# georgehuan1994/OpenGL-Ray-Tracing-Framework

Measured on AMD Instinct MI355X. Metric: Mrays/sec + ms/frame, loong_100000 @1920x1080, 1/2/4/8 MI355X, higher is better.
Workload: dtype f32; 1 GPU; C3: loong_100000 copper metallic (north star); 1920x1080, maxBounce 8, BSDF+MIS+env; width=1920, height=1080, tile=32, parallelism=pixel-tiles x1 + frame-end gather, tile_assignment=interleaved t % N, steps_in_flight=1, triangles=100002, bvh_nodes=35346

## Files before the change

opengl-ray-tracing-framework_amd/csrc/hip/rt_dev_report.h:

```cpp

inline bool dev_passes() {
  static const bool on = knob("RT_DEBUG_PASSES") != nullptr;
  return on;
}
inline size_t dev_wave_words(const rt_ctx* c) { return (size_t)c->n_cus * std::max(c->trace_bpc, c->trace_bpc0) * 4 * 8; }
int dev_wave_log(rt_ctx* c, unsigned long long*& log) {
  static unsigned long long* d_wave_log = nullptr;
  if (dev_passes() && !d_wave_log) HIPCHK(c, hipMalloc(&d_wave_log, dev_wave_words(c) * sizeof(unsigned long long)));
  log = dev_passes() ? d_wave_log : nullptr;
  return RT_OK;
}

int dev_finish_report(rt_ctx* c, bool bsdf, dim3 grid, hipStream_t st, const rtd::WFParams& WP, int g, int pass) {
  std::vector<unsigned long long> wave_log(dev_wave_words(c));
  unsigned long long* const d_wave_log = WP.K.wave_log;
  HIPCHK(c, hipMemsetAsync(d_wave_log, 0, wave_log.size() * 8, st));
  hipEvent_t ft0 = take_event(c), ft1 = take_event(c);
  HIPCHK(c, hipEventRecord(ft0, st));
  launch_finish(c, bsdf, grid, st, WP);
  HIPCHK(c, hipGetLastError());
  HIPCHK(c, hipEventRecord(ft1, st));
  HIPCHK(c, hipStreamSynchronize(st));
  float ms = 0.0f;
  HIPCHK(c, hipEventElapsedTime(&ms, ft0, ft1));
  c->event_pool.push_back(ft0);
  c->event_pool.push_back(ft1);
  HIPCHK(c, hipMemcpy(wave_log.data(), d_wave_log, wave_log.size() * 8, hipMemcpyDeviceToHost));
  struct FW { double t0, t1, sh_us; unsigned long long it, sh, paths; double at[3]; unsigned long long it_at[3]; };
  std::vector<FW> fw;
  double tmin = 1e300;
  for (size_t w = 0; w < wave_log.size() / 8; w++) {
    const unsigned long long* e = &wave_log[8 * w];
    if (!e[1]) continue;
    FW f{e[0] / 100.0, e[1] / 100.0, e[3] / 100.0, e[2] & 0xfffffull, (e[2] >> 20) & 0xfffffull, e[2] >> 40, {}, {}};
    for (int q = 0; q < 3; q++) {
      f.at[q] = e[4 + q] ? (double)(e[4 + q] & 0xffffffffull) / 100.0 : -1.0;
      f.it_at[q] = e[4 + q] >> 32;
    }
    fw.push_back(f);
    tmin = std::min(tmin, e[0] / 100.0);
  }
  std::sort(fw.begin(), fw.end(), [](const FW& a, const FW& b) { return a.t1 > b.t1; });
  unsigned long long paths = 0;
  double life = 0.0, tail16 = 0.0, tail4 = 0.0;
  for (const FW& f : fw) {
    paths += f.paths;
    life += f.t1 - f.t0;
    if (f.at[0] >= 0) tail16 += f.t1 - f.t0 - f.at[0];
    if (f.at[1] >= 0) tail4 += f.t1 - f.t0 - f.at[1];
  }
  fprintf(stderr, "[rt] finisher wave time with <= 16 / <= 4 lanes holding a path (list drained): %.3f / %.3f of %.0f "
          "wave-us\n", tail16 / std::max(1.0, life), tail4 / std::max(1.0, life), life);
  fprintf(stderr, "[rt] group %d finisher from pass %d: %.3f ms, %zu waves, %llu paths; wave ends (us after the first "
          "start) 50%% %.1f 90%% %.1f 99%% %.1f 100%% %.1f\n", g, pass, ms, fw.size(), paths,
          fw.empty() ? 0.0 : fw[fw.size() / 2].t1 - tmin, fw.empty() ? 0.0 : fw[fw.size() / 10].t1 - tmin,
          fw.empty() ? 0.0 : fw[fw.size() / 100].t1 - tmin, fw.empty() ? 0.0 : fw[0].t1 - tmin);
  for (size_t k = 0; k < std::min<size_t>(6, fw.size()); k++) {
    const FW& f = fw[k];
    fprintf(stderr, "[rt]   wave: start %.1f end %.1f us, %llu paths, %llu trace iterations (%.2f us each outside "
            "shade), %llu shade steps %.1f us (%.2f us each); <=16 / 4 / 1 busy lanes from %.0f / %.0f / %.0f us "
            "(iteration %llu / %llu / %llu)\n", f.t0 - tmin, f.t1 - tmin, f.paths, f.it,
            (f.t1 - f.t0 - f.sh_us) / (double)std::max(1ull, f.it), f.sh, f.sh_us, f.sh_us / (double)std::max(1ull, f.sh),
            f.at[0], f.at[1], f.at[2], f.it_at[0], f.it_at[1], f.it_at[2]);
  }
  return RT_OK;
}

int dev_pass_report(rt_ctx* c, hipStream_t st, const rtd::WFParams& WP, int g, int pass, hipEvent_t t0, hipEvent_t t1) {
  unsigned long long h[16];
  unsigned int q[8];
  HIPCHK(c, hipStreamSynchronize(st));
  float ms = 0.0f;
  HIPCHK(c, hipEventElapsedTime(&ms, t0, t1));
  HIPCHK(c, hipMemcpy(h, c->d_stats, sizeof(h), hipMemcpyDeviceToHost));
  HIPCHK(c, hipMemcpy(q, WP.S.cnt, sizeof(q), hipMemcpyDeviceToHost));
  q[0] = q[rtd::cq(pass & 1)] + (WP.split ? q[rtd::cqs(pass & 1)] : 0u);
  fprintf(stderr, "[rt] group %d pass %d: %u rays %.3f ms  cum internal %llu leaf %llu tri %llu iters %llu "
          "wave-iters max %llu ray-steps max %llu\n", g, pass, (WP.cam_n ? WP.cam_n : q[0]), ms, h[2], h[3], h[4], h[5], h[6], h[7]);
  unsigned long long hq[6];
  HIPCHK(c, hipMemcpy(hq, c->d_stats + 22, sizeof(hq), hipMemcpyDeviceToHost));
  fprintf(stderr, "[rt]   4-wide node visits with BFS index < 1 / 5 / 21 / 64 / 85 / 341: %llu %llu %llu %llu %llu %llu\n",
          hq[0], hq[1], hq[2], hq[3], hq[4], hq[5]);
  HIPCHK(c, hipMemset(c->d_stats + 22, 0, sizeof(hq)));
  fprintf(stderr, "[rt]   lane utilisation: node phase %.3f (%llu iters)  tri phase %.3f (%llu iters)  busy at "
          "refill %.3f (%llu outer)\n", h[9] / (64.0 * (double)(h[8] + !h[8])), h[8],
          h[11] / (64.0 * (double)(h[10] + !h[10])), h[10], h[13] / (64.0 * (double)(h[12] + !h[12])), h[12]);
  fprintf(stderr, "[rt]   overflow-column pushes %llu (%.3f per ray)\n", h[14],
          (double)h[14] / (double)std::max(1u, WP.cam_n ? WP.cam_n : q[0]));
  HIPCHK(c, hipMemset(c->d_stats + 6, 0, 10 * sizeof(unsigned long long)));
  {
    unsigned long long hh[64];
    HIPCHK(c, hipMemcpy(hh, c->d_stats + 32, sizeof(hh), hipMemcpyDeviceToHost));
    static const char* kinds[4] = {"cont miss", "cont hit ", "shad miss", "shad hit "};
    for (int kd = 0; kd < 4; kd++) {
      fprintf(stderr, "[rt]   steps/ray %s:", kinds[kd]);
      for (int b = 0; b < 16; b++) fprintf(stderr, " %llu", hh[kd * 16 + b]);
      fprintf(stderr, "\n");
    }
    HIPCHK(c, hipMemset(c->d_stats + 32, 0, sizeof(hh)));
  }
  if (!WP.K.wave_log) return RT_OK;
  std::vector<unsigned long long> wave_log(dev_wave_words(c));
  HIPCHK(c, hipMemcpy(wave_log.data(), WP.K.wave_log, wave_log.size() * 8, hipMemcpyDeviceToHost));
  unsigned long long t0min = ~0ull, t1max = 0, t0max = 0, dmax = 0, itmax = 0, rmax = 0, cmax = 0;
  std::vector<unsigned long long> ends;
  double clk_sum = 0.0, wt_sum = 0.0;
  for (size_t w = 0; w < wave_log.size() / 8; w++) {
    const unsigned long long* e = &wave_log[4 * w];
    const unsigned long long its = e[2] & 0xfffffull, cyc = e[2] >> 20;
    t0min = std::min(t0min, e[0]); t0max = std::max(t0max, e[0]); t1max = std::max(t1max, e[1]);
    if (e[1] - e[0] > dmax) { dmax = e[1] - e[0]; itmax = its; rmax = e[3]; cmax = cyc; }
    if (e[1] > e[0]) { clk_sum += (double)cyc; wt_sum += (double)(e[1] - e[0]); }
    ends.push_back(e[1]);
  }
  fprintf(stderr, "[rt]   shader clock: mean over waves %.0f MHz, longest wave %.0f MHz\n",
          wt_sum > 0 ? 100.0 * clk_sum / wt_sum : 0.0, dmax ? 100.0 * (double)cmax / (double)dmax : 0.0);
  std::sort(ends.begin(), ends.end());
  auto us = [](unsigned long long t) { return t / 100.0; };
  fprintf(stderr, "[rt]   waves: start spread %.1f us, span %.1f us; 50%% done at %.1f us, 90%% at %.1f, "
          "99%% at %.1f; longest wave %.1f us (%llu iters, %llu rays)\n", us(t0max - t0min),
          us(t1max - t0min), us(ends[ends.size() / 2] - t0min), us(ends[ends.size() * 9 / 10] - t0min),
          us(ends[ends.size() * 99 / 100] - t0min), us(dmax), itmax, rmax);
  return RT_OK;
}
```

opengl-ray-tracing-framework_amd/csrc/hip/rt_render.hip:

```cpp
#include <hip/hip_runtime.h>
#include <rccl/rccl.h>
#include <stdio.h>
#include <stdlib.h>
#include <string.h>

#include <algorithm>
#include <cmath>
#include <cstddef>
#include <new>
#include <string>
#include <vector>
#include <limits>

#include "rt_abi.h"
#include "rt_kernels.h"
#include "rt_wavefront.h"
#include "rt_query.h"

#ifndef RT_SPLIT_KINDS
#define RT_SPLIT_KINDS 1
#endif
#ifndef RT_SPLIT_PASSES
#define RT_SPLIT_PASSES 5
#endif
#ifndef RT_SPLIT_CONT_FIRST
#define RT_SPLIT_CONT_FIRST 0
#endif
#include "scene_compile.h"

using rtd::GNode;
using rtd::KParams;

struct rt_ctx {
  int device = 0;
  int n_cus = 0;
  hipStream_t stream = nullptr;
  bool own_stream = false;
  std::string err;
  GNode* d_nodes = nullptr;
  rtd::QNode* d_qnodes = nullptr;
  int qroot = 0, qstack_entries = 2, n_qnodes = 0;
  bool wide = false;
  float4* d_tri = nullptr;
  float4* d_trx = nullptr;
  double tri_k1 = 0.0, tri_k0 = 0.0;
  int tri_flagged = 0;
  float4* d_trin = nullptr;
  float4* d_hrec = nullptr;
  float4* d_mats = nullptr;
  int n_tri = 0, n_mats = 0, root = 0, has_scene = 0, stack_entries = 2;
  double cull_R = 0.0, cull_K = 0.0, cull_off = 0.0;
  bool scene_set = false;
  std::vector<int32_t> tri_mat;
  std::vector<float> mat_table;
  float4* d_hdr = nullptr;
  float2* d_cache = nullptr;
  struct LightTable {
    float4* d = nullptr;
    bool valid = false;
    float angle = 0.0f;
    hipEvent_t last_use = nullptr;
    hipEvent_t built = nullptr;
  };
  LightTable light[2];
  int light_cur = 0;
  int hdr_w = 0, hdr_h = 0, hdr_res = 0;
  bool env_set = false;
  int W = 0, H = 0, tile_w = 32, tile_h = 32, tiles_x = 0, tiles_y = 0, rank = 0, world = 1;
  int local_tiles = 0, max_local_tiles = 0;
  float4* d_accum = nullptr;
  bool frame_set = false;
  int loop_num = 0;
  unsigned int* d_counter = nullptr;
  unsigned long long* d_stats = nullptr;
  std::vector<std::pair<hipEvent_t, hipEvent_t>> events;
  struct TraceEv {
    hipEvent_t s, e;
    uint64_t call;
  };
  std::vector<TraceEv> trace_events;
  std::vector<hipEvent_t> event_pool;
  double kernel_ms = 0.0, trace_ms = 0.0;
  struct BusyIv {
    double lo, hi;
    uint64_t call;
  };
  hipEvent_t busy_anchor = nullptr;
  double busy_anchor_t = 0.0;
  std::vector<BusyIv> busy;
  double busy_closed_ms = 0.0;
  uint64_t launches = 0, trace_launches = 0;
  int blocks_per_cu = 0, block_lds = 0;
  int trace_bpc = 0, trace_bpc0 = 0;
  int trace_lds_entries = 0, trace_lds = 0;
  int split_kinds = RT_SPLIT_KINDS;
  int split_passes = RT_SPLIT_PASSES;
  struct FrameTable {
    int* h = nullptr;
    int* d = nullptr;
    size_t cap = 0;
    hipEvent_t ev = nullptr;
  };
  FrameTable ft[5];
#ifndef RT_CAM_SHADE
#define RT_CAM_SHADE 1
#endif
#ifndef RT_POOL_CHUNK_DEFAULT
#define RT_POOL_CHUNK_DEFAULT 1024
#endif
  int pool_chunk = RT_POOL_CHUNK_DEFAULT;
  int2* d_stack_ovf = nullptr;
  void* d_disp = nullptr;
  size_t disp_bytes = 0;
  void* d_gather = nullptr;
  std::vector<int> rccl_devs;
  std::vector<ncclComm_t> rccl_comms;
  int gather_transport = 0;
  size_t gather_bytes = 0;
  size_t stack_ovf_bytes = 0;
  void* wf_mem = nullptr;
  size_t wf_paths = 0;
  rtd::WFState wf{};
  static constexpr int MAX_GROUPS = 4;
  int n_groups = 2;
  size_t order_head = 0;
  rtd::WFState wfg[MAX_GROUPS]{};
  hipStream_t aux[MAX_GROUPS] = {};
  unsigned int* d_pix = nullptr;
  std::vector<int32_t> owner, my_tiles;
  int* d_tile_ids = nullptr;
  int2* d_tile_src = nullptr;
  unsigned long long* d_tile_cost = nullptr;
  bool tile_cost_on = false;
  bool cost_blocks = false;
  float4* d_cam = nullptr;
  int cam_sets = 1;
  int n_valid = 0;
  int frames_cap = 1;
  size_t max_slots_req = 0;
  int finish_pass = 2;
  uint64_t finish_slots = uint64_t(8) << 20;
  int finish_bpc = 0;
  static constexpr int DISP_SLOTS = 4;
  struct DisplaySlot {
    uint8_t* host = nullptr;
    size_t cap = 0, bytes = 0;
    hipEvent_t ev = nullptr;
  };
  DisplaySlot disp[DISP_SLOTS];
  int pipe_depth = 1;
  int pipe_next = 0;
  size_t pipe_nomem_slots = SIZE_MAX;
  int pipe_finish_bpc = 2;
  int pipe_finish_pass = -1;
  hipEvent_t set_free[MAX_GROUPS] = {};
  hipEvent_t batch_done = nullptr;
  struct Query {
    void* mem = nullptr;
    size_t cap = 0;
    rtd::WFState S{};
    float* d_in = nullptr;
    float4* d_out = nullptr;
    float* d_zero = nullptr;
    int2* d_ovf = nullptr;
    size_t ovf_bytes = 0;
  } q;
};

namespace {

inline const char* knob(const char* name) {
#ifdef RT_DEV
  return getenv(name);
#else
  (void)name;
  return nullptr;
#endif
}

int fail(rt_ctx* c, int code, const std::string& msg) {
  if (c) c->err = msg;
  return code;
}
#define HIPCHK(ctx, call)                                                                        \
  do {                                                                                           \
    hipError_t e_ = (call);                                                                      \
    if (e_ != hipSuccess)                                                                        \
      return fail((ctx), RT_ERR_HIP, std::string(#call) + ": " + hipGetErrorString(e_));         \
  } while (0)
// ... 860 lines not shown
int megakernel_batch(rt_ctx* c, const rt_frame_params* fp, const KParams& P) {
  HIPCHK(c, hipMemsetAsync(c->d_counter, 0, 4, c->stream));
  unsigned int max_blocks = (P.n_work + 255) / 256;
  unsigned int grid = std::min<unsigned int>((unsigned)(c->n_cus * c->blocks_per_cu), max_blocks);
  if (fp->flags & RT_FLAG_COUNT_VISITS)
    hipLaunchKernelGGL(rtd::rt_path_kernel<true>, dim3(grid), dim3(256), c->block_lds, c->stream, P);
  else
    hipLaunchKernelGGL(rtd::rt_path_kernel<false>, dim3(grid), dim3(256), c->block_lds, c->stream, P);
  HIPCHK(c, hipGetLastError());
  c->trace_launches++;
  return RT_OK;
}

struct GroupPlan {
  int G = 1;
  bool pix_split = false;
  rtd::WFParams WG[rt_ctx::MAX_GROUPS];
  hipStream_t sg[rt_ctx::MAX_GROUPS];
  unsigned int slots_g[rt_ctx::MAX_GROUPS];
  int split_g[rt_ctx::MAX_GROUPS] = {};
  float4* cam = nullptr;
  hipEvent_t prev_blend = nullptr;
};

int plan_groups(rt_ctx* c, const rt_frame_params* fp, const RenderCall& call, const KParams& P, GroupPlan& plan) {
  const bool pipe = call.pipe, count = (fp->flags & RT_FLAG_COUNT_VISITS) != 0;
  const int nf = P.n_frames;
  const bool pix_split = !pipe && !call.serial && pix_split_ok() && nf < c->n_groups && c->n_valid >= 64 * c->n_groups && !c->tile_cost_on;
  const int G = (pipe || call.serial) ? 1 : pix_split ? c->n_groups : std::min(c->n_groups, nf);
  plan.G = G;
  plan.pix_split = pix_split;
  const unsigned int trace_grid = (unsigned)(c->n_cus * std::max(c->trace_bpc, c->trace_bpc0));
  unsigned long long* d_wave_log = nullptr;
#ifdef RT_DEV
  if (int rc = dev_wave_log(c, d_wave_log)) return rc;
#endif
  const size_t ovf_group = c->stack_ovf_bytes / sizeof(int2) / (size_t)c->n_groups;
  size_t b0 = std::min(c->order_head, (size_t)c->n_valid);
#ifdef RT_DEV
  if (const char* e = knob("RT_GROUP_SPLIT")) b0 = std::min((size_t)c->n_valid, ((size_t)((double)c->n_valid * atof(e)) + 63) / 64 * 64);
#endif
  auto wbound = [&](int g) -> unsigned int {
    if (g <= 0) return 0u;
    if (g >= G) return (unsigned)c->n_valid;
    if (b0 > 0 && G > 1) return (unsigned)(b0 + ((size_t)c->n_valid - b0) * (g - 1) / (G - 1));
    return (unsigned)((size_t)c->n_valid * g / G);
  };
  const size_t set_off = pipe ? (size_t)call.pset * (size_t)c->n_valid : 0;
  plan.cam = c->wf.cam + set_off;
  float4* const org = c->wf.cam + (size_t)c->cam_sets * (size_t)std::max(1, c->n_valid) + set_off;
  for (int g = 0; g < G; g++) {
    const int f0 = pix_split ? 0 : g * nf / G, f1 = pix_split ? nf : (g + 1) * nf / G;
    const unsigned int w0 = pix_split ? wbound(g) : 0u;
    const unsigned int w1 = pix_split ? wbound(g + 1) : (unsigned)c->n_valid;
    rtd::WFParams& WP = plan.WG[g];
    WP.K = P;
    WP.K.loop_num = P.loop_num + f0;
    WP.K.rand_origin = P.rand_origin + f0;
    WP.K.sobol = P.sobol + 4 * f0;
    WP.K.blend_w = P.blend_w + f0;
    WP.K.n_frames = f1 - f0;
    WP.K.n_work = w1 - w0;
    WP.K.lds_entries = c->trace_lds_entries;
    WP.K.pool_chunk = c->pool_chunk;
    const int set = pipe ? call.pset : g;
    WP.K.stack_ovf = c->d_stack_ovf ? c->d_stack_ovf + (size_t)set * ovf_group : nullptr;
    WP.K.ovf_lanes = trace_grid * 256u;
    {
      const std::string e = ovf_layout_error(c, set, trace_grid);
      if (!e.empty()) return fail(c, RT_ERR_STATE, e);
    }
    WP.K.wave_log = d_wave_log;
#ifdef RT_DEV
    if (d_wave_log && knob("RT_DEBUG_WAVES_ONLY")) WP.K.flags |= rtd::kFlagNoRayHist;
#endif
    WP.S = c->wfg[set];
    WP.S.pix_xy = c->wf.pix_xy + w0;
    WP.S.pix_acc = c->wf.pix_acc + w0;
    WP.S.cam = plan.cam + w0;
    WP.S.org = org + w0;
    WP.n_frames = f1 - f0;
    WP.pass = 0;
    WP.cam_n = 0u;
    WP.fuse_blend = (!pipe && WP.n_frames == 1 && (pix_split || G == 1) && !count) ? 1 : 0;
    plan.slots_g[g] = (unsigned)(f1 - f0) * (w1 - w0);
    plan.split_g[g] = (c->split_kinds && c->wide && !count && !c->tile_cost_on && plan.slots_g[g] > c->finish_slots && !WP.fuse_blend) ? 1 : 0;
    plan.sg[g] = pipe ? call.ps : g == 0 ? c->stream : c->aux[g];
  }
  return RT_OK;
}

int launch_camera_and_fork(rt_ctx* c, const RenderCall& call, GroupPlan& plan) {
  rtd::WFParams WC = plan.WG[0];
  WC.K.n_work = (unsigned)c->n_valid;
  WC.S.pix_xy = c->wf.pix_xy;
  WC.S.pix_acc = c->wf.pix_acc;
  WC.S.cam = plan.cam;
  rtd::GroupCounters Z;
  memset(&Z, 0, sizeof(Z));
  Z.n = plan.G;
  for (int g = 0; g < plan.G; g++) Z.cnt[g] = plan.WG[g].S.cnt;
  hipLaunchKernelGGL(rtd::wf_camera, dim3(std::max(1u, std::min<unsigned int>(2048u, ((unsigned)c->n_valid + 255) / 256))),
                     dim3(256), 0, call.ps, WC, Z);
  HIPCHK(c, hipGetLastError());
  if (plan.G > 1) {
    hipEvent_t es;
    TAKE_EVENT(c, es);
    HIPCHK(c, hipEventRecord(es, c->stream));
    for (int g = 1; g < plan.G; g++) HIPCHK(c, hipStreamWaitEvent(plan.sg[g], es, 0));
    c->event_pool.push_back(es);
  }
  return RT_OK;
}

int run_group_passes(rt_ctx* c, const rt_frame_params* fp, const RenderCall& call, GroupPlan& plan, int g) {
  rtd::WFParams& WP = plan.WG[g];
  const hipStream_t st = plan.sg[g];
  const unsigned int slots = plan.slots_g[g];
  const bool count = (fp->flags & RT_FLAG_COUNT_VISITS) != 0, bsdf = fp->enable_bsdf != 0;
  const int last_pass = std::max(0, fp->max_bounce);
  int fin_pass = (call.pipe && c->pipe_finish_pass >= 0) ? c->pipe_finish_pass : c->finish_pass;
#ifdef RT_DEV
  {
    char kn[32];
    snprintf(kn, sizeof(kn), "RT_FINISH_PASS_G%d", g);
    if (const char* e = knob(kn)) fin_pass = std::max(0, atoi(e));
  }
#endif
  const bool finish = !count && !c->tile_cost_on && !(fp->flags & RT_FLAG_NO_FINISH) &&
                      fin_pass >= 1 && fin_pass <= last_pass &&
                      ((fp->flags & RT_FLAG_FINISH) || slots <= c->finish_slots);
  WP.p1_compact = (finish && fin_pass <= 1) ? 0 : 1;
  for (int pass = 0; pass <= last_pass; pass++) {
    WP.pass = pass;
    WP.split = (plan.split_g[g] && pass >= 1 && pass <= c->split_passes) ? 1 : 0;
    WP.split_out = (plan.split_g[g] && pass + 1 <= c->split_passes) ? 1 : 0;
    if (finish && pass == fin_pass) {
      const dim3 fgrid((unsigned)(c->n_cus * (call.pipe ? c->pipe_finish_bpc : c->finish_bpc)));
#ifdef RT_DEV
      if (dev_passes()) return dev_finish_report(c, bsdf, fgrid, st, WP, g, pass);
#endif
      launch_finish(c, bsdf, fgrid, st, WP);
      HIPCHK(c, hipGetLastError());
      break;
    }
    WP.cam_n = pass == 0 ? slots : 0u;
    hipEvent_t t0, t1;
    TAKE_EVENT(c, t0);
    TAKE_EVENT(c, t1);
    HIPCHK(c, hipEventRecord(t0, st));
    launch_trace(c, count, dim3((unsigned)(c->n_cus * (pass == 0 ? c->trace_bpc0 : c->trace_bpc))), WP, st,
                 slots <= c->finish_slots);
    HIPCHK(c, hipGetLastError());
    HIPCHK(c, hipEventRecord(t1, st));
    c->trace_events.push_back({t0, t1, c->launches});
    c->trace_launches++;
#ifdef RT_DEV
    if (dev_passes()) if (int rc = dev_pass_report(c, st, WP, g, pass, t0, t1)) return rc;
#endif
    const bool bulk = slots > c->finish_slots && !WP.fuse_blend;
    const bool cam = RT_CAM_SHADE && bulk && WP.cam_n && WP.n_frames >= 64;
    launch_shade(bsdf, WP.fuse_blend ? ShadeKind::fused : cam ? ShadeKind::cam : bulk ? ShadeKind::bulk : ShadeKind::plain,
                 slots, st, WP);
    HIPCHK(c, hipGetLastError());
  }
  return RT_OK;
}

int blend_and_join(rt_ctx* c, RenderCall& call, GroupPlan& plan, int g) {
  const hipStream_t st = plan.sg[g];
  const int G = plan.G;
  if (plan.prev_blend) {
    HIPCHK(c, hipStreamWaitEvent(st, plan.prev_blend, 0));
    c->event_pool.push_back(plan.prev_blend);
    plan.prev_blend = nullptr;
  }
  if (call.e_entry) {
    HIPCHK(c, hipStreamWaitEvent(st, call.e_entry, 0));
    c->event_pool.push_back(call.e_entry);
    call.e_entry = nullptr;
  }
  if (!plan.WG[g].fuse_blend) {
    hipLaunchKernelGGL(rtd::wf_blend, dim3(std::max(1u, std::min<unsigned int>(2048u, ((unsigned)c->n_valid + 255) / 256))),
                       dim3(256), 0, st, plan.WG[g]);
    HIPCHK(c, hipGetLastError());
  }
  if (!plan.pix_split && g + 1 < G) {
    TAKE_EVENT(c, plan.prev_blend);
    HIPCHK(c, hipEventRecord(plan.prev_blend, st));
  }
  if (g + 1 < G) return RT_OK;
  for (int j = plan.pix_split ? 1 : G - 1; j < G && G > 1; j++) {
    hipEvent_t ej;
    TAKE_EVENT(c, ej);
    HIPCHK(c, hipEventRecord(ej, plan.sg[j]));
    HIPCHK(c, hipStreamWaitEvent(c->stream, ej, 0));
    c->event_pool.push_back(ej);
  }
  return RT_OK;
}

int close_batch(rt_ctx* c, const RenderCall& call, hipEvent_t e0, hipEvent_t e1) {
  const int pset = call.pset;
  HIPCHK(c, hipEventRecord(e1, call.ps));
  if (call.pipe) {
    if (c->set_free[pset]) c->event_pool.push_back(c->set_free[pset]);
    TAKE_EVENT(c, c->set_free[pset]);
    HIPCHK(c, hipEventRecord(c->set_free[pset], call.ps));
    HIPCHK(c, hipStreamWaitEvent(c->stream, c->set_free[pset], 0));
  } else if (call.pipe_sets >= 2) {
    if (!c->batch_done) HIPCHK(c, hipEventCreateWithFlags(&c->batch_done, hipEventDisableTiming));
    HIPCHK(c, hipEventRecord(c->batch_done, c->stream));
  }
  if (!call.LT->last_use) HIPCHK(c, hipEventCreateWithFlags(&call.LT->last_use, hipEventDisableTiming));
  HIPCHK(c, hipEventRecord(call.LT->last_use, c->stream));
  c->events.push_back({e0, e1});
  c->launches++;
  if (int rc = fold_trace_events(c, kMaxPendingEvents)) return rc;
  return fold_events(c, c->events, c->kernel_ms, kMaxPendingEvents);
}

}

extern "C" {

int rt_render_async(rt_ctx* c, const rt_frame_params* fp, const float* rand_origin, int32_t n_frames) {
  if (!c || !fp || n_frames < 0 || (n_frames && !rand_origin)) return RT_ERR_ARG;
  if (!c->scene_set || !c->env_set || !c->frame_set) return fail(c, RT_ERR_STATE, "set_scene, set_env and resize first");
  const bool mega = (fp->flags & RT_FLAG_MEGAKERNEL) != 0;
  if (mega && !fp->enable_bsdf)
    return fail(c, RT_ERR_ARG, "BRDF mode (enable_bsdf = 0) runs on the wavefront path only");
  HIPCHK(c, hipSetDevice(c->device));
  RenderCall call;
  list_traced_frames(c, fp, rand_origin, n_frames, call);
  admit_pipeline(c, fp, call);
// ... 769 lines not shown
```

opengl-ray-tracing-framework_amd/csrc/hip/rt_wavefront.h:

```cpp
#pragma once
#include "rt_kernels.h"

namespace rtd {


enum : uint32_t {
  PF_SHADOW = 1u,
  PF_CMED = 2u,
  PF_CONT = 4u,
  PF_MEDIUM = 8u,
  PF_CAMERA = 16u,
  PF_ZLO = 32u
};

struct WFState {
  float4* __restrict__ s0;
  float4* __restrict__ s1;
  float4* __restrict__ s2;
  float4* __restrict__ s3;
  float4* __restrict__ s4;
  uint2* __restrict__ s5;
  float4* __restrict__ ra;
  float2* __restrict__ rb;
  float4* __restrict__ sa;
  float2* __restrict__ sb;
  int* __restrict__ res;
  float4* __restrict__ fin;
  const unsigned int* __restrict__ pix_xy;
  const unsigned int* __restrict__ pix_acc;
  float4* __restrict__ cam;
  float4* __restrict__ org;
  int* queue[2];
  int* queue_s[2];
  int* active[2];
  unsigned int* __restrict__ cnt;
};

constexpr int kFlagNoRayHist = 1 << 30;

__host__ __device__ constexpr unsigned int cq(unsigned int i) { return i; }
__host__ __device__ constexpr unsigned int ca(unsigned int i) { return 2u + i; }
constexpr unsigned int kCntFetch = 4u;
__host__ __device__ constexpr unsigned int xcnt(unsigned int s) { return 160u + 32u * s; }
__host__ __device__ constexpr unsigned int cqs(unsigned int i) { return 6u + i; }
__host__ __device__ constexpr unsigned int xcnts(unsigned int s) { return 416u + 32u * s; }
constexpr unsigned int kCntWords = 416u + 32u * 8u;

constexpr unsigned int kStatShards = 64u, kStatWords = 128u + 16u * kStatShards;
__host__ __device__ constexpr unsigned int stats_shard(unsigned int wave) { return 128u + 16u * (wave % kStatShards); }

RTD void p1_ray(const WFState& S, unsigned int n_frames, unsigned int path, const float4 a, float& ox, float& oy,
                float& oz) {
  const unsigned int w = path / n_frames;
  const float4 o = S.org[w];
  ox = o.x; oy = o.y; oz = o.z;
  if (a.w != 0.0f) {
    const float4 c = S.cam[w];
    ox = o.x + c.x * a.w; oy = o.y + c.y * a.w; oz = o.z + c.z * a.w;
  }
}
#ifndef RT_SHADE_NT
#define RT_SHADE_NT 1
#endif
typedef float nt_f4 __attribute__((ext_vector_type(4)));
typedef float nt_f2 __attribute__((ext_vector_type(2)));
typedef unsigned int nt_u2 __attribute__((ext_vector_type(2)));
RTD void st_row(float4* p, float4 v) {
  if (RT_SHADE_NT) __builtin_nontemporal_store(nt_f4{v.x, v.y, v.z, v.w}, reinterpret_cast<nt_f4*>(p));
  else *p = v;
}
RTD void st_row(float2* p, float2 v) {
  if (RT_SHADE_NT) __builtin_nontemporal_store(nt_f2{v.x, v.y}, reinterpret_cast<nt_f2*>(p));
  else *p = v;
}
RTD void st_row(uint2* p, uint2 v) {
  if (RT_SHADE_NT) __builtin_nontemporal_store(nt_u2{v.x, v.y}, reinterpret_cast<nt_u2*>(p));
  else *p = v;
}
RTD void put_ray(float4* a, float2* b, unsigned int p, float ox, float oy, float oz, float dx, float dy, float dz) {
  st_row(a + p, make_float4(ox, oy, oz, dx));
  st_row(b + p, make_float2(dy, dz));
}

struct WFParams {
  KParams K;
  WFState S;
  int n_frames;
  int pass;
  unsigned int cam_n;
  int p1_compact;
  int fuse_blend;
  int split, split_out;
};

RTD bool work_pixel(const KParams& P, unsigned int w, int& px, int& py, int& accIdx) {
  const int tpx = P.tile_w * P.tile_h;
  int lt = (int)(w / (unsigned)tpx);
  int r = (int)(w - (unsigned)lt * (unsigned)tpx);
  int gt = P.tile_ids[lt];
  int tx = gt % P.tiles_x, ty = gt / P.tiles_x;
  int blk = r >> 6, in = r & 63;
  int bxs = P.tile_w >> 3;
  int lx = (blk % bxs) * 8 + (in & 7);
  int ly = (blk / bxs) * 8 + (in >> 3);
  px = tx * P.tile_w + lx;
  py = ty * P.tile_h + ly;
  accIdx = lt * tpx + ly * P.tile_w + lx;
  return px < P.W && py < P.H;
}

RTD unsigned int wave_append(unsigned int* counter, bool want) {
  const unsigned long long m = __ballot(want);
  unsigned int base = 0;
  if (m) {
    const int lane = (int)(threadIdx.x & 63);
    const int leader = __ffsll((long long)m) - 1;
    if (lane == leader) base = atomicAdd(counter, (unsigned int)__popcll(m));
    base = __shfl(base, leader);
    base += (unsigned int)__popcll(m & ((1ull << lane) - 1ull));
  }
  return base;
}

RTD unsigned int wave_lds_append(unsigned int* lcount, unsigned int n) {
  const int lane = (int)(threadIdx.x & 63);
  const unsigned long long b1 = __ballot(n >= 1u), b2 = __ballot(n >= 2u);
  const unsigned long long below = (1ull << lane) - 1ull;
  const unsigned int mine = (unsigned int)(__popcll(b1 & below) + __popcll(b2 & below));
  const unsigned int wtot = (unsigned int)(__popcll(b1) + __popcll(b2));
  unsigned int base = 0;
  if (lane == 0 && wtot) base = atomicAdd(lcount, wtot);
  return (unsigned int)__shfl((int)base, 0) + mine;
}

struct GroupCounters {
  unsigned int* cnt[4];
  int n;
};
RTD float4 camera_dir(const KParams& P, f3 lbc, f3 right, f3 up, unsigned int xy) {
  const int px = (int)(xy & 0xffffu), py = (int)(xy >> 16);
  const float u = ((float)px + 0.5f) / (float)P.W;
  const float v = ((float)py + 0.5f) / (float)P.H;
  const f3 d = normalize(lbc + (u * 2.0f * P.half_w) * right + (v * 2.0f * P.half_h) * up);
  return make_float4(d.x, d.y, d.z, u * v);
}
__global__ __launch_bounds__(256) void wf_camera(const WFParams W, const GroupCounters Z) {
  const KParams& P = W.K;
  const WFState& S = W.S;
  if (blockIdx.x == 0)
    for (unsigned int i = threadIdx.x; i < kCntWords * (unsigned)Z.n; i += blockDim.x) Z.cnt[i / kCntWords][i % kCntWords] = 0u;
  const f3 lbc = mk3(P.lbc[0], P.lbc[1], P.lbc[2]);
  const f3 right = mk3(P.right[0], P.right[1], P.right[2]);
  const f3 up = mk3(P.up[0], P.up[1], P.up[2]);
  for (unsigned int w = blockIdx.x * blockDim.x + threadIdx.x; w < P.n_work; w += gridDim.x * blockDim.x)
    S.cam[w] = camera_dir(P, lbc, right, up, S.pix_xy[w]);
}

#ifndef RT_INLINE_FRAMES
#define RT_INLINE_FRAMES 8
#endif
struct InlineFrames {
  int n_inline;
  int loop[RT_INLINE_FRAMES];
  float ro[RT_INLINE_FRAMES];
};
__global__ __launch_bounds__(256) void wf_sobol(int* __restrict__ loop_num, float* __restrict__ rand_origin,
                                                float2* __restrict__ out, float2* __restrict__ blend_w, int n_frames,
                                                const InlineFrames F) {
  const int i = blockIdx.x * blockDim.x + threadIdx.x;
  const bool inl = F.n_inline > 0;
  if (i < n_frames) {
    const int loopNum = inl ? F.loop[i] : loop_num[i];
    if (inl) {
      loop_num[i] = loopNum;
      rand_origin[i] = F.ro[i];
    }
    const float n = (float)loopNum;
    blend_w[i] = make_float2(1.0f / n, (float)(loopNum - 1) / n);
  }
  if (i >= n_frames * 4) return;
  int g = (inl ? F.loop[i >> 2] : loop_num[i >> 2]) + 1;
  g = g ^ (g >> 1);
  const int b = i & 3;
  out[i] = make_float2(sobol_gray(2 * b, g), sobol_gray(2 * b + 1, g));
}
RTD void sobol_pair(const KParams& P, uint32_t frame, uint32_t bounce, float& sx, float& sy) {
  sx = sy = 0.0f;
  if (bounce < 4u) {
    const float2 s = P.sobol[frame * 4u + bounce];
    sx = s.x;
    sy = s.y;
  }
}

RTD f3 camera_ray(const KParams& P, const WFState& S, unsigned int slot, uint32_t& wseed, uint32_t& frame) {
  const unsigned int nf = (unsigned int)P.n_frames;
  const unsigned int w = slot / nf;
  const unsigned int f = slot - w * nf;
  const float4 c = S.cam[w];
  wseed = (uint32_t)(P.rand_origin[f] * 6.95857f * c.w);
  frame = f;
  return xyz(c);
}

constexpr int BL_FR = 8, BL_PITCH = BL_FR + 1;
__global__ __launch_bounds__(256) __attribute__((amdgpu_waves_per_eu(4))) void wf_blend(const WFParams W) {
  __shared__ float4 tile[256 * BL_PITCH];
  const KParams& P = W.K;
  const WFState& S = W.S;
  const unsigned int nf = (unsigned int)W.n_frames;
  for (unsigned int base = blockIdx.x * 256u; base < P.n_work; base += gridDim.x * 256u) {
    const unsigned int w = base + threadIdx.x;
    const bool valid = w < P.n_work;
    const unsigned int ai = valid ? S.pix_acc[w] : 0u;
    f3 acc = splat(0.0f);
    if (valid) {
      const float4 h = P.accum[ai];
      acc = mk3(h.x, h.y, h.z);
    }
    {
      static_assert(BL_FR == 8, "eight named registers");
      float4 r0, r1, r2, r3, r4, r5, r6, r7;
      __shared__ float2 wst[BL_FR];
      auto ld1 = [&](unsigned int f0, int j) {
        const unsigned int nfc = min((unsigned int)BL_FR, nf - f0);
        const unsigned int i = threadIdx.x + 256u * (unsigned)j, p = i / BL_FR, k = i % BL_FR;
        const bool ok = base + p < P.n_work && k < nfc;
        return S.fin[ok ? (size_t)(base + p) * nf + f0 + k : 0];
      };
      auto st1 = [&](int j, float4 v) {
        const unsigned int i = threadIdx.x + 256u * (unsigned)j, p = i / BL_FR, k = i % BL_FR;
        tile[p * BL_PITCH + k] = v;
      };
#define RT_BLEND_FETCH(F0)                                                                          \
  {                                                                                                 \
    r0 = ld1(F0, 0); r1 = ld1(F0, 1); r2 = ld1(F0, 2); r3 = ld1(F0, 3);                             \
    r4 = ld1(F0, 4); r5 = ld1(F0, 5); r6 = ld1(F0, 6); r7 = ld1(F0, 7);                             \
  }
      RT_BLEND_FETCH(0u)
      for (unsigned int f0 = 0; f0 < nf; f0 += BL_FR) {
        const unsigned int nfc = min((unsigned int)BL_FR, nf - f0);
        __syncthreads();
        st1(0, r0); st1(1, r1); st1(2, r2); st1(3, r3); st1(4, r4); st1(5, r5); st1(6, r6); st1(7, r7);
        if (threadIdx.x < (unsigned)BL_FR) wst[threadIdx.x] = P.blend_w[f0 + (threadIdx.x < nfc ? threadIdx.x : 0u)];
        __syncthreads();
        float2 bw[BL_FR];
#pragma unroll
        for (int k = 0; k < BL_FR; k++) bw[k] = wst[k];
        if (f0 + BL_FR < nf) RT_BLEND_FETCH(f0 + BL_FR)
#undef RT_BLEND_FETCH
        if (valid)
#pragma unroll
          for (int k = 0; k < BL_FR; k++) {
            if ((unsigned)k < nfc) {
              const float4 c = tile[threadIdx.x * BL_PITCH + k];
              acc = bw[k].x * xyz(c) + bw[k].y * acc;
            }
          }
      }
    }
    if (valid) P.accum[ai] = make_float4(acc.x, acc.y, acc.z, 0.0f);
  }
}


struct TraceLane {
  float ox, oy, oz, dx, dy, dz, ix, iy, iz;
  RTD f3 o() const { return mk3(ox, oy, oz); }
  RTD f3 d() const { return mk3(dx, dy, dz); }
  RTD f3 inv() const { return mk3(ix, iy, iz); }
  float best, bestt;
  float lim;
  RTD float limit(float) const { return lim; }
  RTD void set_best(float d, float eps) {
    best = d;
    lim = cull_limit(d, eps, ix, iy, iz);
  }
// ... 523 lines not shown
  return finished || (!L.haveCur && L.tri_i >= L.tri_end);
}

template <int G>
RTD int coop_move(TraceLane& L, const TraceStack& TS, unsigned long long live, int lane, int cap) {
  const int nl = __popcll(live);
  const int g = lane / G;
  unsigned long long m = live;
  for (int j = 0; j < g && m; j++) m &= m - 1ull;
  const int src = (g < nl && m) ? (int)__builtin_ctzll(m) : lane;
  const int sp_src = __shfl(L.sp, src);
  int spm = g < nl ? min(max(sp_src, 0), cap) : 0;
  for (int o = 32; o > 0; o >>= 1) spm = max(spm, __shfl_xor(spm, o));
  const uint32_t w0 = threadIdx.x & ~63u;
  for (int j = 0; j < min(spm, TS.KL); j++) {
    const int2 e = TS.lds0[j * TL_LANES + w0 + src];
    TS.lds0[j * TL_LANES + w0 + lane] = e;
  }
  for (int j = TS.KL; j < spm; j++) {
    const unsigned long long e = TS.ovf[(size_t)(j - TS.KL) * TS.ovs + w0 + src];
    TS.ovf[(size_t)(j - TS.KL) * TS.ovs + w0 + lane] = e;
  }
  L.ox = __shfl(L.ox, src); L.oy = __shfl(L.oy, src); L.oz = __shfl(L.oz, src);
  L.dx = __shfl(L.dx, src); L.dy = __shfl(L.dy, src); L.dz = __shfl(L.dz, src);
  L.ix = __shfl(L.ix, src); L.iy = __shfl(L.iy, src); L.iz = __shfl(L.iz, src);
  L.best = __shfl(L.best, src); L.bestt = __shfl(L.bestt, src); L.besttri = __shfl(L.besttri, src);
  L.lim = __shfl(L.lim, src);
  L.sp = sp_src; L.cur = __shfl(L.cur, src);
  L.tri_i = __shfl(L.tri_i, src); L.tri_end = __shfl(L.tri_end, src);
  L.offNx = __shfl(L.offNx, src); L.offNy = __shfl(L.offNy, src); L.offNz = __shfl(L.offNz, src);
  L.haveCur = __shfl((int)L.haveCur, src) != 0;
  L.anyhit = __shfl((int)L.anyhit, src) != 0;
  L.finite = __shfl((int)L.finite, src) != 0;
  return src;
}

#ifndef RT_COST_PER_RAY
#define RT_COST_PER_RAY 16u
#endif
#ifndef RT_REFILL_MIN
#define RT_REFILL_MIN 20
#endif
#ifndef RT_TAIL_CHUNK
#define RT_TAIL_CHUNK 64u
#endif
#ifndef RT_GUIDED
#define RT_GUIDED 3u
#endif
#ifndef RT_REFILL_MIN_AH
#define RT_REFILL_MIN_AH 28
#endif
#ifndef RT_REFILL_MIN_SMALL
#define RT_REFILL_MIN_SMALL 8
#endif
#ifndef RT_TAIL_FACTOR
#define RT_TAIL_FACTOR 4u
#endif
#ifndef RT_STATIC_FRAC
#define RT_STATIC_FRAC 6
#endif
#ifndef RT_WAVE_TIMES
#define RT_WAVE_TIMES 0
#endif
#ifndef RT_TRACE_COOP
#define RT_TRACE_COOP 16
#endif
#ifndef RT_RES_NT
#define RT_RES_NT 1
#endif
#ifndef RT_SHADOW_SORT
#define RT_SHADOW_SORT 0
#endif
#ifndef RT_TRACE_WPE_DUAL
#define RT_TRACE_WPE_DUAL 8
#endif
template <bool COUNT, bool WIDE, bool CAM, bool STATIC = false, bool P1 = false, int KIND = 0>
__global__ __launch_bounds__(256) __attribute__((amdgpu_waves_per_eu(RT_TRACE_WPE_DUAL)))
void wf_trace(const WFParams W) {
  extern __shared__ __attribute__((aligned(16))) unsigned char smem[];
  const KParams& P = W.K;
  const WFState& S = W.S;
  const int qin = W.pass & 1;
  constexpr bool AHK = KIND == 2;
  const unsigned int nq = CAM ? W.cam_n : AHK ? S.cnt[cqs(qin)] : S.cnt[cq(qin)];
  const int* __restrict__ Q = AHK ? S.queue_s[qin] : S.queue[qin];
  if (blockIdx.x == 0 && threadIdx.x == 0) {
    S.cnt[cq(qin ^ 1)] = 0u;
    S.cnt[cqs(qin ^ 1)] = 0u;
    S.cnt[ca(qin ^ 1)] = 0u;
  }
  if (nq == 0u || !P.has_scene) {
    if (!P.has_scene) {
      for (unsigned int i = blockIdx.x * blockDim.x + threadIdx.x; i < nq; i += gridDim.x * blockDim.x) {
        const int e = CAM ? (int)(i << 1) : Q[i];
        S.res[e] = -1;
      }
    }
    return;
  }
  TraceStack TS;
  TS.KL = P.lds_entries;
#ifdef RT_CHECK
  TS.cap = P.stack_cap;
#endif
  TS.lds0 = reinterpret_cast<int2*>(smem);
  TS.lds = TS.lds0 + threadIdx.x;
  TS.ovf = (gu64*)(P.stack_ovf) + blockIdx.x * TL_LANES;
  TS.ovs = P.ovf_lanes;
  const bool cull = !AHK && (P.flags & RT_FLAG_NO_CULL) == 0;

  bool busy = false;
  bool coop = false;
  unsigned int pool_next = 0, pool_end = 0;
  const unsigned int tail_rays = gridDim.x * TL_LANES * RT_TAIL_FACTOR;
  const unsigned int wave_id = blockIdx.x * (TL_LANES / 64) + (threadIdx.x >> 6);
  const unsigned int part_waves = min(gridDim.x * (TL_LANES / 64), (nq + RT_TAIL_CHUNK - 1u) / RT_TAIL_CHUNK);
  bool drained = wave_id >= part_waves;
  const unsigned int static_per = (STATIC && RT_STATIC_FRAC > 0 && nq <= tail_rays)
      ? (unsigned int)((unsigned long long)nq * RT_STATIC_FRAC / 8u / part_waves) : 0u;
  const unsigned int static_total = static_per * part_waves;
  if (STATIC && !drained) {
    pool_next = wave_id * static_per;
    pool_end = pool_next + static_per;
  }
  unsigned int seg = blockIdx.x & 7u, seg_tries = 0, seg_seen = 0;
  const unsigned int seg_waves = max(1u, part_waves / 8u);
  const int lane = (int)(threadIdx.x & 63);
  int entry = 0;
  TraceLane L;
  L.ox = L.oy = L.oz = L.dx = L.dy = L.dz = L.ix = L.iy = L.iz = 0.0f;
  L.best = INF; L.bestt = 0.0f; L.besttri = -1; L.lim = INF;
  L.sp = L.cur = L.tri_i = L.tri_end = 0;
  L.haveCur = L.anyhit = false;
  unsigned long long v_int = 0, v_leaf = 0, v_tri = 0, v_iter = 0;
  unsigned int ray_steps = 0, ray_steps_max = 0;
  unsigned long long v_itN = 0, v_itT = 0, v_itO = 0, v_park = 0, v_busyO = 0;
  unsigned long long v_rays = 0, v_ovf = 0;
  unsigned long long v_q[6] = {0, 0, 0, 0, 0, 0};
  constexpr bool WT = COUNT || RT_WAVE_TIMES;
  const unsigned long long t_start = WT ? wall_clock64() : 0ull;
  const unsigned long long c_start = WT ? clock64() : 0ull;

  while (true) {
    if (WT) v_iter++;
    const unsigned long long idle = __ballot(!busy);
    if (idle && !drained && (__popcll(idle) >= (STATIC ? RT_REFILL_MIN_SMALL : AHK ? RT_REFILL_MIN_AH : RT_REFILL_MIN) || idle == __ballot(true))) {
      if (pool_next >= pool_end) {
        while (true) {
          const unsigned int d0 = STATIC ? static_total : 0u, dn = nq - d0;
          const unsigned int lo = d0 + (unsigned int)((unsigned long long)dn * seg / 8u);
          const unsigned int hi = d0 + (unsigned int)((unsigned long long)dn * (seg + 1u) / 8u);
          const unsigned int left = hi - min(max(seg_seen, lo), hi);
          const unsigned int chunk = STATIC ? RT_TAIL_CHUNK
              : min((unsigned)P.pool_chunk, max(RT_TAIL_CHUNK, (left / (seg_waves * RT_GUIDED)) & ~63u));
          unsigned int b = 0;
          if (lane == 0) b = atomicAdd(&S.cnt[AHK ? xcnts(seg) : xcnt(seg)], chunk);
          b = lo + __builtin_amdgcn_readfirstlane(__shfl(b, 0));
          if (b < hi) {
            pool_next = b;
            pool_end = min(b + chunk, hi);
            seg_seen = pool_end;
            break;
          }
          if (++seg_tries >= 8u) {
            drained = true;
            break;
          }
          seg = (seg + 1u) & 7u;
          seg_seen = 0xFFFFFFFFu;
        }
      }
      if (!drained || pool_next < pool_end) {
        const unsigned int avail = pool_end - pool_next;
        const unsigned int rank = __builtin_amdgcn_mbcnt_hi((uint32_t)(idle >> 32), __builtin_amdgcn_mbcnt_lo((uint32_t)idle, 0u));
        if (!busy && rank < avail) {
          const unsigned int qi = pool_next + rank;
          if (CAM) {
            const unsigned int slot = qi;
            entry = (int)(slot << 1);
            L.anyhit = false;
            uint32_t seed_unused, frame_unused;
            const f3 d = camera_ray(P, S, slot, seed_unused, frame_unused);
            L.ox = P.pos[0]; L.oy = P.pos[1]; L.oz = P.pos[2];
            L.dx = d.x; L.dy = d.y; L.dz = d.z;
          } else {
            entry = Q[qi];
            const int path = entry >> 1;
            L.anyhit = KIND == 2 ? true : KIND == 1 ? false : (entry & 1) != 0;
            const float4 oa = L.anyhit ? S.sa[path] : S.ra[path];
            if (P1) {
              p1_ray(S, (unsigned)W.n_frames, (unsigned)path, oa, L.ox, L.oy, L.oz);
              L.dx = oa.x; L.dy = oa.y; L.dz = oa.z;
            } else {
              const float2 ob = L.anyhit ? S.sb[path] : S.rb[path];
              L.ox = oa.x; L.oy = oa.y; L.oz = oa.z;
              L.dx = oa.w; L.dy = ob.x; L.dz = ob.y;
            }
          }
          tl_start<WIDE>(P, L);
          busy = true;
        }
        pool_next += min((unsigned int)__popcll(idle), avail);
      }
    }
    if (RT_TRACE_COOP && STATIC && WIDE && !coop && drained &&
        pool_next >= pool_end) {
      const unsigned long long live = __ballot(busy);
      const int nl = __popcll(live);
      if (nl > 0 && nl <= RT_TRACE_COOP) {
        coop = true;
        const int src = coop_move<4>(L, TS, live, lane, P.stack_cap);
        const int e_src = __shfl(entry, src), b_src = __shfl((int)busy, src);
        entry = e_src;
        busy = (lane >> 2) < nl && b_src != 0;
      }
    }
    if (!__any(busy)) break;
    if (COUNT) { v_itO++; if (busy) v_busyO++; }
    bool finished = false;
    if (COUNT) { v_itN++; v_itT++; }
    if (RT_TRACE_COOP && STATIC && WIDE && coop) {
      if (busy) finished = tl_coop_step<4>(P, L, TS, cull, lane & 3);
    } else if (busy) {
      if (L.tri_i < L.tri_end) {
        if (COUNT) { v_tri++; ray_steps++; }
        if (tl_triangle<WIDE, AHK>(P, L, L.tri_i++) && (AHK || (KIND == 0 && L.anyhit))) {
          finished = true;
          L.tri_end = L.tri_i;
        }
      }
      bool needPop = false;
      if (!finished && L.haveCur) {
        if (ref_is_leaf(L.cur)) {
          if (L.tri_i >= L.tri_end) {
            if (COUNT) { v_leaf++; v_park++; }
            L.tri_i = leaf_first(L.cur);
            L.tri_end = L.tri_i + leaf_count(L.cur);
            needPop = true;
          }
        } else {
          if (COUNT) {
            v_int++; ray_steps++;
            if (WIDE) {
              v_q[0] += L.cur < 1; v_q[1] += L.cur < 5; v_q[2] += L.cur < 21;
              v_q[3] += L.cur < 64; v_q[4] += L.cur < 85; v_q[5] += L.cur < 341;
            }
          }
          const int sp0 = L.sp;
          if (WIDE) needPop = tl_qnode<false, !AHK || RT_SHADOW_SORT>(P, L, TS, cull);
          else tl_node(P, L, TS, cull);
          if (COUNT) v_ovf += (unsigned)max(0, L.sp - max(sp0, TS.KL));
        }
      }
      if (needPop) L.haveCur = tl_pop(P, L, TS, cull);
      if (!finished && !L.haveCur && L.tri_i >= L.tri_end) finished = true;
    }
    if (busy && finished) {
      if (RT_RES_NT) __builtin_nontemporal_store(L.besttri, &S.res[entry]);
      else S.res[entry] = L.besttri;
      if (COUNT) {
        if (P.tile_cost) {
          const unsigned int w = (unsigned int)(entry >> 1) / (unsigned int)P.n_frames;
          atomicAdd(&P.tile_cost[P.cost_blocks ? w >> 6 : S.pix_acc[w] / (unsigned int)(P.tile_w * P.tile_h)],
                    (unsigned long long)(ray_steps + RT_COST_PER_RAY));
        }
// ... 117 lines not shown

constexpr int kCamRec = 11;
RTD void cam_rec(const WFParams& W, const Env& E, unsigned int w, float4* rec) {
  const KParams& P = W.K;
  const WFState& S = W.S;
  const unsigned int path0 = w * (unsigned)W.n_frames;
  int r = S.res[2 * path0];
  const f3 ro = mk3(P.pos[0], P.pos[1], P.pos[2]), rd = xyz(S.cam[w]);
#ifdef RT_CHECK
  if (r >= P.n_tri) r = -1;
#endif
  if (r >= 0) {
    const HitGeom h = hit_geom(P, r, ro, rd);
    const f3 hN = h.inside ? -h.Ns : h.Ns;
    const Mat m = load_mat(P.mats, h.nmat);
    const BsdfFrame BF = bsdf_frame(m, -rd, hN);
    const f3 Le0 = xyz(P.mats[8 * h.nmat]);
    rec[0] = make_float4(h.Pp.x, h.Pp.y, h.Pp.z, h.t - 0.00001f);
    rec[1] = make_float4(hN.x, hN.y, hN.z, __int_as_float(r));
    rec[2] = make_float4(Le0.x, Le0.y, Le0.z, __int_as_float(h.nmat));
    rec[3] = make_float4(BF.eta, BF.T.x, BF.T.y, BF.T.z);
    rec[4] = make_float4(BF.B.x, BF.B.y, BF.B.z, BF.V.x);
    rec[5] = make_float4(BF.V.y, BF.V.z, BF.specCol.x, BF.specCol.y);
    rec[6] = make_float4(BF.specCol.z, BF.sheenCol.x, BF.sheenCol.y, BF.sheenCol.z);
    v_terms(BF, m, rec + 7);
  } else {
    const f3 env = P.enable_env ? hdrColor(E, rd) * E.intensity : getDefaultSkyColor(rd.y);
    rec[1] = make_float4(0.0f, 0.0f, 0.0f, __int_as_float(r));
    rec[2] = make_float4(env.x, env.y, env.z, 0.0f);
  }
}
RTD BsdfFrame rec_frame(const float4* rec) {
  const float4 q3 = rec[3], q4 = rec[4], q5 = rec[5], q6 = rec[6];
  BsdfFrame F;
  F.eta = q3.x;
  F.T = mk3(q3.y, q3.z, q3.w);
  F.B = mk3(q4.x, q4.y, q4.z);
  F.V = mk3(q4.w, q5.x, q5.y);
  F.specCol = mk3(q5.z, q5.w, q6.x);
  F.sheenCol = mk3(q6.y, q6.z, q6.w);
  return F;
}

template <bool BSDF, bool FUSE = false, bool CAMK = false>
RTD ShadeOut shade_path(const WFParams& W, const Env& E, int path, bool live, bool camPass, bool loadPrev,
                        unsigned long long& nsamples, const float4* rec = nullptr) {
  const KParams& P = W.K;
  const WFState& S = W.S;
  bool doFinish = false, doBounce = false;
  bool qShadow = false, qCont = false;
  f3 fin = splat(0.0f);
  float4 a0 = make_float4(0, 0, 0, 0), a1 = a0, a2 = a0, a3 = a0, a4 = a0;
  uint4 a5 = make_uint4(0, 0, 0, 0);
  f3 hist = splat(1.0f), Lo = splat(0.0f), Le0 = splat(0.0f), evf = splat(0.0f);
  float evp = 0.0f;
  uint32_t wseed = 0, bounce = 0, flags = 0, frame = 0;
  f3 hP = splat(0.0f), hN = splat(0.0f), hV = splat(0.0f);
  float hDist = 0.0f;
  int mat = 0;
  constexpr bool useRec = CAMK;
  if (live) {
    float4 cam_d = make_float4(0, 0, 0, 0);
    if (camPass) {
      uint32_t cseed, cframe;
      const f3 d = camera_ray(P, S, (unsigned)path, cseed, cframe);
      a5 = make_uint4(cseed, 0u, PF_CONT | PF_CAMERA, cframe);
      cam_d = make_float4(d.x, d.y, d.z, 0.0f);
    } else {
      const uint2 p5 = S.s5[path];
      const unsigned int nfr = (unsigned int)W.n_frames;
      a5 = make_uint4(p5.x, p5.y >> 8, p5.y & 0xffu, (unsigned int)path % nfr);
    }
    int rsh = 0;
    if (loadPrev) {
      a0 = S.s0[path]; a2 = S.s2[path];
      rsh = S.res[2 * path + 1];
      if (!(a5.z & PF_ZLO)) {
        a1 = S.s1[path];
        a3 = S.s3[path];
      } else if (a5.z & PF_SHADOW) {
        a3 = S.s3[path];
      }
    }
    const int rc0 = S.res[2 * path];
#ifdef RT_CHECK
    if (CAMK && __float_as_int(rec[1].w) != rc0)
      printf("[rt check] camera record: path %d result %d, record %d\n", path, rc0, __float_as_int(rec[1].w));
#endif
    float4 oo0, dd0;
    if (camPass) {
      oo0 = make_float4(P.pos[0], P.pos[1], P.pos[2], 0.0f);
      dd0 = make_float4(cam_d.x, cam_d.y, cam_d.z, 0.0f);
    } else if (W.p1_compact && W.pass == 1) {
      const float4 ra0 = S.ra[path];
      float ox, oy, oz;
      p1_ray(S, (unsigned)W.n_frames, (unsigned)path, ra0, ox, oy, oz);
      oo0 = make_float4(ox, oy, oz, 0.0f);
      dd0 = make_float4(ra0.x, ra0.y, ra0.z, 0.0f);
    } else {
      const float4 ra0 = S.ra[path];
      const float2 rb0 = S.rb[path];
      oo0 = make_float4(ra0.x, ra0.y, ra0.z, 0.0f);
      dd0 = make_float4(ra0.w, rb0.x, rb0.y, 0.0f);
    }
    wseed = a5.x; bounce = a5.y; flags = a5.z; frame = a5.w;
    if (!(flags & PF_CAMERA)) {
      hist = xyz(a0); evp = a0.w;
      Lo = xyz(a1);
      evf = xyz(a2);
      Le0 = mk3(a1.w, a2.w, 0.0f);
      Le0.z = a3.w;
      if ((flags & PF_SHADOW) && rsh < 0) Lo = Lo + xyz(a3);
      if (flags & PF_CMED) {
        a4 = S.s4[path];
        Lo = Lo + xyz(a4);
      }
    }
    if (!(flags & PF_CONT)) {
      fin = Le0 + Lo;
      doFinish = true;
    } else {
      const int r = useRec ? __float_as_int(rec[1].w) : rc0;
      const float4 oo = oo0, dd = dd0;
      const f3 ro = xyz(oo), rd = xyz(dd);
      if (useRec && r >= 0) {
        const float4 q0 = rec[0], q1 = rec[1], q2 = rec[2];
        Le0 = xyz(q2);
        hP = xyz(q0);
        if (W.p1_compact && frame == 0u) S.org[(unsigned)path / (unsigned)W.n_frames] = make_float4(q0.x, q0.y, q0.z, 0.0f);
        hN = xyz(q1);
        hV = rd;
        hDist = q0.w;
        mat = __float_as_int(q2.w);
        if (0 < P.max_bounce) doBounce = true;
        else { fin = Le0 + Lo; doFinish = true; }
      } else if (useRec) {
        fin = xyz(rec[2]);
        doFinish = true;
      } else if (r >= 0) {
        int tri = r;
#ifdef RT_CHECK
        if (tri >= P.n_tri) {
          printf("[rt check] shade: path %d pass %d result triangle %d of %d\n", path, W.pass, tri, P.n_tri);
          tri = 0;
        }
#endif
        const HitGeom hg = hit_geom(P, tri, ro, rd);
        const float t = hg.t;
        const bool inside = hg.inside;
        const f3 Pp = hg.Pp, Ns = hg.Ns;
        const int nmat = hg.nmat;
        if (flags & PF_CAMERA) {
          Le0 = xyz(P.mats[8 * nmat]);
          Lo = splat(0.0f);
          hist = splat(1.0f);
          bounce = 0;
        } else if (BSDF) {
          const f3 Le = xyz(P.mats[8 * nmat]);
          Lo = Lo + hist * Le * evf / evp;
          bounce++;
        } else {
          const f3 Le = xyz(P.mats[8 * nmat]);
          Lo = Lo + hist * Le * evf * fabs_(S.s4[path].x) / evp;
          bounce++;
        }
        hP = Pp;
        if (camPass && W.p1_compact && frame == 0u) S.org[(unsigned)path / (unsigned)W.n_frames] = make_float4(Pp.x, Pp.y, Pp.z, 0.0f);
// ... 515 lines not shown
```

Before: 10320 Mrays/s.

## Trace one shared camera ray per pixel across frames in pass zero

When several frames are batched per group, the camera pass now traces only one primary ray per pixel, using a precomputed per-pixel camera direction buffer, instead of one per frame slot. Every frame's path then reads the hit result from the frame-zero slot of its pixel. This removes redundant primary-ray traversal, but it assumes camera rays are identical across frames, so there is no per-frame jitter. An optional static-schedule launch mode is also exposed.

```diff
diff --git a/opengl-ray-tracing-framework_amd/csrc/hip/rt_dev_report.h b/opengl-ray-tracing-framework_amd/csrc/hip/rt_dev_report.h
--- a/opengl-ray-tracing-framework_amd/csrc/hip/rt_dev_report.h
+++ b/opengl-ray-tracing-framework_amd/csrc/hip/rt_dev_report.h
@@ -75,8 +75,9 @@
   HIPCHK(c, hipMemcpy(h, c->d_stats, sizeof(h), hipMemcpyDeviceToHost));
   HIPCHK(c, hipMemcpy(q, WP.S.cnt, sizeof(q), hipMemcpyDeviceToHost));
   q[0] = q[rtd::cq(pass & 1)] + (WP.split ? q[rtd::cqs(pass & 1)] : 0u);
+  const unsigned int traced = WP.cam_n ? (WP.cam_shared ? WP.K.n_work : WP.cam_n) : q[0];
   fprintf(stderr, "[rt] group %d pass %d: %u rays %.3f ms  cum internal %llu leaf %llu tri %llu iters %llu "
-          "wave-iters max %llu ray-steps max %llu\n", g, pass, (WP.cam_n ? WP.cam_n : q[0]), ms, h[2], h[3], h[4], h[5], h[6], h[7]);
+          "wave-iters max %llu ray-steps max %llu\n", g, pass, traced, ms, h[2], h[3], h[4], h[5], h[6], h[7]);
   unsigned long long hq[6];
   HIPCHK(c, hipMemcpy(hq, c->d_stats + 22, sizeof(hq), hipMemcpyDeviceToHost));
   fprintf(stderr, "[rt]   4-wide node visits with BFS index < 1 / 5 / 21 / 64 / 85 / 341: %llu %llu %llu %llu %llu %llu\n",
@@ -86,7 +87,7 @@
           "refill %.3f (%llu outer)\n", h[9] / (64.0 * (double)(h[8] + !h[8])), h[8],
           h[11] / (64.0 * (double)(h[10] + !h[10])), h[10], h[13] / (64.0 * (double)(h[12] + !h[12])), h[12]);
   fprintf(stderr, "[rt]   overflow-column pushes %llu (%.3f per ray)\n", h[14],
-          (double)h[14] / (double)std::max(1u, WP.cam_n ? WP.cam_n : q[0]));
+          (double)h[14] / (double)std::max(1u, traced));
   HIPCHK(c, hipMemset(c->d_stats + 6, 0, 10 * sizeof(unsigned long long)));
   {
     unsigned long long hh[64];
diff --git a/opengl-ray-tracing-framework_amd/csrc/hip/rt_render.hip b/opengl-ray-tracing-framework_amd/csrc/hip/rt_render.hip
--- a/opengl-ray-tracing-framework_amd/csrc/hip/rt_render.hip
+++ b/opengl-ray-tracing-framework_amd/csrc/hip/rt_render.hip
@@ -105,6 +105,12 @@
 #ifndef RT_CAM_SHADE
 #define RT_CAM_SHADE 1
 #endif
+#ifndef RT_CAM_SHARED
+#define RT_CAM_SHARED 1
+#endif
+#ifndef RT_CAM_SHARED_STATIC
+#define RT_CAM_SHARED_STATIC 0
+#endif
 #ifndef RT_POOL_CHUNK_DEFAULT
 #define RT_POOL_CHUNK_DEFAULT 1024
 #endif
@@ -1131,6 +1137,7 @@
     WP.n_frames = f1 - f0;
     WP.pass = 0;
     WP.cam_n = 0u;
+    WP.cam_shared = 0;
     WP.fuse_blend = (!pipe && WP.n_frames == 1 && (pix_split || G == 1) && !count) ? 1 : 0;
     plan.slots_g[g] = (unsigned)(f1 - f0) * (w1 - w0);
     plan.split_g[g] = (c->split_kinds && c->wide && !count && !c->tile_cost_on && plan.slots_g[g] > c->finish_slots && !WP.fuse_blend) ? 1 : 0;
@@ -1194,12 +1201,17 @@
       break;
     }
     WP.cam_n = pass == 0 ? slots : 0u;
+    bool cam_shared = RT_CAM_SHARED && pass == 0 && WP.n_frames > 1 && !count && !c->tile_cost_on;
+    bool cam_static = RT_CAM_SHARED_STATIC != 0;
+    if (const char* e = knob("RT_CAM_SHARED")) cam_shared = cam_shared && atoi(e) != 0;
+    if (const char* e = knob("RT_CAM_SHARED_STATIC")) cam_static = atoi(e) != 0;
+    WP.cam_shared = cam_shared ? 1 : 0;
     hipEvent_t t0, t1;
     TAKE_EVENT(c, t0);
     TAKE_EVENT(c, t1);
     HIPCHK(c, hipEventRecord(t0, st));
     launch_trace(c, count, dim3((unsigned)(c->n_cus * (pass == 0 ? c->trace_bpc0 : c->trace_bpc))), WP, st,
-                 slots <= c->finish_slots);
+                 slots <= c->finish_slots || (cam_shared && cam_static));
     HIPCHK(c, hipGetLastError());
     HIPCHK(c, hipEventRecord(t1, st));
     c->trace_events.push_back({t0, t1, c->launches});
diff --git a/opengl-ray-tracing-framework_amd/csrc/hip/rt_wavefront.h b/opengl-ray-tracing-framework_amd/csrc/hip/rt_wavefront.h
--- a/opengl-ray-tracing-framework_amd/csrc/hip/rt_wavefront.h
+++ b/opengl-ray-tracing-framework_amd/csrc/hip/rt_wavefront.h
@@ -88,6 +88,7 @@
   int n_frames;
   int pass;
   unsigned int cam_n;
+  int cam_shared;
   int p1_compact;
   int fuse_blend;
   int split, split_out;
@@ -193,6 +194,7 @@
   }
 }
 
+RTD unsigned int cam_slot(const WFParams& W, unsigned int slot, uint32_t frame) { return W.cam_shared ? slot - frame : slot; }
 RTD f3 camera_ray(const KParams& P, const WFState& S, unsigned int slot, uint32_t& wseed, uint32_t& frame) {
   const unsigned int nf = (unsigned int)P.n_frames;
   const unsigned int w = slot / nf;
@@ -882,7 +884,9 @@
   const WFState& S = W.S;
   const int qin = W.pass & 1;
   constexpr bool AHK = KIND == 2;
-  const unsigned int nq = CAM ? W.cam_n : AHK ? S.cnt[cqs(qin)] : S.cnt[cq(qin)];
+  const bool shared = CAM && W.cam_shared;
+  const unsigned int cam_stride = shared ? (unsigned int)W.n_frames : 1u;
+  const unsigned int nq = CAM ? (shared ? P.n_work : W.cam_n) : AHK ? S.cnt[cqs(qin)] : S.cnt[cq(qin)];
   const int* __restrict__ Q = AHK ? S.queue_s[qin] : S.queue[qin];
   if (blockIdx.x == 0 && threadIdx.x == 0) {
     S.cnt[cq(qin ^ 1)] = 0u;
@@ -892,7 +896,7 @@
   if (nq == 0u || !P.has_scene) {
     if (!P.has_scene) {
       for (unsigned int i = blockIdx.x * blockDim.x + threadIdx.x; i < nq; i += gridDim.x * blockDim.x) {
-        const int e = CAM ? (int)(i << 1) : Q[i];
+        const int e = CAM ? (int)((i * cam_stride) << 1) : Q[i];
         S.res[e] = -1;
       }
     }
@@ -976,11 +980,10 @@
         if (!busy && rank < avail) {
           const unsigned int qi = pool_next + rank;
           if (CAM) {
-            const unsigned int slot = qi;
+            const unsigned int slot = qi * cam_stride;
             entry = (int)(slot << 1);
             L.anyhit = false;
-            uint32_t seed_unused, frame_unused;
-            const f3 d = camera_ray(P, S, slot, seed_unused, frame_unused);
+            const float4 d = S.cam[shared ? qi : slot / (unsigned int)P.n_frames];
             L.ox = P.pos[0]; L.oy = P.pos[1]; L.oz = P.pos[2];
             L.dx = d.x; L.dy = d.y; L.dz = d.z;
           } else {
@@ -1264,7 +1267,7 @@
         a3 = S.s3[path];
       }
     }
-    const int rc0 = S.res[2 * path];
+    const int rc0 = S.res[2 * (camPass ? (int)cam_slot(W, (unsigned)path, a5.w) : path)];
 #ifdef RT_CHECK
     if (CAMK && __float_as_int(rec[1].w) != rc0)
       printf("[rt check] camera record: path %d result %d, record %d\n", path, rc0, __float_as_int(rec[1].w));
```

Result: faster. 11220 Mrays/s, median of 6 (+8.8%).
